# nghiapq77/face-recognition-cpp-tensorrt

Measured on AMD Instinct MI355X. Metric: faces/sec end-to-end (detect+embed+match), 640x640 batch=32, 1M gallery, higher is better.
Workload: dtype f16 MFMA recogniser convs (fp32 accumulate) + fp32-accurate detector (fp32 MFMA, fp16 hi/lo-split MFMA for the 64-channel 3x3 convs) + int8-screened coarse scan (fp16 MFMA on exactly widened int8 rows) + exact f32 re-rank match (bit-identical to the exact f32 scan)

## Files before the change

### face-recognition-cpp-tensorrt_amd/csrc/frt_kernels.h

```cpp
#pragma once
#include <hip/hip_runtime.h>
#include <stdint.h>

#include <vector>

#include "../../include/frt.h"
#include "frt_faces.hpp"

typedef _Float16 half_t;
typedef _Float16 half8 __attribute__((ext_vector_type(8)));
typedef _Float16 half4 __attribute__((ext_vector_type(4)));
typedef float floatx16 __attribute__((ext_vector_type(16)));
typedef float floatx4 __attribute__((ext_vector_type(4)));

constexpr int FRT_MAX_DEVICES = 32;
inline bool frt_first_use_on_device(bool (&done)[FRT_MAX_DEVICES]) {
    int d = 0;
    (void)hipGetDevice(&d);
    d &= FRT_MAX_DEVICES - 1;
    if (done[d]) return false;
    done[d] = true;
    return true;
}

// ... 230 lines not shown
    int linear;
    int nt;
    int R;
    int n_img;
    int nslot;
    int threads;
};
struct StripTables {
    int period = 0;
    int ppx = 0;
    int stride = 0;
    std::vector<int> data;
};
constexpr int strip_table_stride(const StripGeometry &g) { return g.nslot * g.threads + g.nt * 64 + (g.compact ? g.nt * 4 : g.nt * 32); }
StripTables strip_tables(const StripGeometry &g);
enum ConvFamily { CONV_SMALL, CONV_KS, CONV_C64, CONV_S2, CONV_STRIP };
struct ConvPlan {
    int family = CONV_STRIP;
    int row = 0;
    const char *label = "";
    int R = 0, n_img = 1;
    int M = 0;
    bool uses_scx = false;
    int se_row = -1;
    const char *se_label = nullptr;
    bool se_fused() const { return se_row >= 0; }
    void take_se_tail() { row = se_row; label = se_label; }
};
struct ConvRow {
    const char *label;
// ... 1 lines not shown
    int se_row;
};
inline void conv_plan_row(ConvPlan &p, int family, const ConvRow *table, int row) {
    p.family = family;
    p.row = row;
    p.label = table[row].label;
}
inline void conv_plan_se_twin(ConvPlan &p, const ConvRow *table, const ConvMfmaArgs &a) {
    if (table[p.row].se_row < 0 || a.mode != EPI_BN_ADD_BN || !a.se_pool || !a.sc || !a.out1) return;
    p.se_row = table[p.row].se_row;
    p.se_label = table[p.se_row].label;
}
ConvPlan conv_plan(const ConvMfmaArgs &a);
bool conv_strip_geometry(const ConvMfmaArgs &a, const ConvPlan &p, StripGeometry &g);
void conv_strip_tables_warm(const ConvMfmaArgs &a, const ConvPlan &p);
void launch_conv_mfma(const ConvMfmaArgs &a, const ConvPlan &p, hipStream_t s);
bool conv_se_fits_device();
bool plan_small(const ConvMfmaArgs &a, ConvPlan &p);
void launch_small(const ConvMfmaArgs &a, const ConvPlan &p, hipStream_t s);
bool plan_ks(const ConvMfmaArgs &a, ConvPlan &p);
void launch_ks(const ConvMfmaArgs &a, const ConvPlan &p, hipStream_t s);
bool plan_c64(const ConvMfmaArgs &a, ConvPlan &p);
void launch_c64(const ConvMfmaArgs &a, const ConvPlan &p, hipStream_t s);
bool plan_s2(const ConvMfmaArgs &a, ConvPlan &p);
void launch_s2(const ConvMfmaArgs &a, const ConvPlan &p, hipStream_t s);
struct ArcInputArgs {
    const float *x;
    const float *w;
    const float *s0, *b0;
    const float *slope;
// ... 37 lines not shown
```

### face-recognition-cpp-tensorrt_amd/csrc/kernels_arc.hip

```cpp
#include "frt_kernels.h"
#include "frt_se_device.h"

#include <array>
#include <map>
#include <mutex>
#include <stdexcept>
#include <string>
#include <type_traits>
#include <utility>
#include <vector>

namespace {

__device__ __forceinline__ int swz(int row, int chunk) { return chunk ^ ((row >> 1) & 7); }

template <int WCO, int WPX, int NSTAGE>
__global__ __launch_bounds__(256) void conv_glds_kernel(ConvMfmaArgs p) {
    constexpr int BCO = WCO * 64, BPX = WPX * 64;
    constexpr int CO_CH = BCO * 8 / 256, PX_CH = BPX * 8 / 256;
    constexpr int LPT = CO_CH + PX_CH;
    constexpr int STAGE_HALFS = (BCO + BPX) * 64;
    extern __shared__ __attribute__((aligned(16))) char smem[];
    half_t *ring = reinterpret_cast<half_t *>(smem);

// ... 878 lines not shown
    if (plan_c64(a, p)) return p;
    if (plan_s2(a, p)) return p;
    plan_strip(a, p);
    return p;
}

bool conv_strip_geometry(const ConvMfmaArgs &a, const ConvPlan &p, StripGeometry &g) {
    if (p.family != CONV_STRIP || !kStripGeometry[p.row]) return false;
    g = kStripGeometry[p.row](a, p);
    return true;
}

void conv_strip_tables_warm(const ConvMfmaArgs &a, const ConvPlan &p) {
    StripGeometry g;
    if (conv_strip_geometry(a, p, g)) (void)strip_tab_device(g);
}

StripTables strip_tables(const StripGeometry &g) {
    const int H = g.H, W = g.W, NT = g.nt, R = g.R, T = g.threads, P = H * W, S = NT * 32;
    auto bad = [](const char *what) { throw std::runtime_error(std::string("strip tables: ") + what); };
    if (H < 1 || W < 1 || NT < 1 || R < 1 || g.n_img < 1 || g.nslot < 1 || (T != 128 && T != 256)) bad("geometry");
    StripTables t;
    t.stride = strip_table_stride(g);
    const int o_pbase = g.nslot * T, o_tail = o_pbase + NT * 64;
    const int patch_bytes = g.nslot * T * 16, PROW = 144;
    const int Wp = g.compact ? W : W + 2;
    if (g.compact) {
        int a = P, b = S;
        while (b) { const int c = a % b; a = b; b = c; }
        t.period = P / a;
// ... 128 lines not shown
```

### face-recognition-cpp-tensorrt_amd/csrc/kernels_arc_s2.hip

```cpp
#include "frt_kernels.h"
#include "frt_se_device.h"

#include <type_traits>

namespace {

constexpr int PROW = 144;

__device__ constexpr int kSub[9] = {0, 0, 0, 0, 1, 2, 2, 3, 3};
__device__ constexpr int kDr[9] = {0, 0, 1, 1, 0, 0, 1, 0, 0};
__device__ constexpr int kDc[9] = {0, 1, 0, 1, 0, 0, 0, 0, 1};
__device__ constexpr int kLen[4] = {4, 1, 2, 2};
__device__ constexpr int kRowPar[4] = {1, 0, 1, 0};
__device__ constexpr int kColPar[4] = {1, 0, 0, 1};

template <int NT, int PP, bool SEP = false, bool SCF = false>
__global__ __launch_bounds__(256, 1) void conv_s2_kernel(ConvMfmaArgs p, int R, int n_img, int linear) {
    constexpr int PLANE_B = PP * 4096;
    constexpr int LA = 2, WR = 3, BFD = 2;
    extern __shared__ __attribute__((aligned(16))) char smem[];
    const int tid = threadIdx.x, lane = tid & 63, wave = tid >> 6;
    const int r = lane & 31, hi = lane >> 5;
    const int H = p.H, W = p.W, Ho = p.Ho, Wo = p.Wo, Wq = Wo + 1;
    const int NPp = n_img * (R + 1) * Wq;
    const int strips_per_img = Ho / R;
    const int n_valid = n_img * R * Wo;

    const int n_co_tiles = p.Cout >> 7;
    const int nblk = gridDim.x, bq = nblk >> 3, brem = nblk & 7;
    const int xcd = blockIdx.x & 7, slot = blockIdx.x >> 3;
    const int lid = (xcd < brem ? xcd * (bq + 1) : brem * (bq + 1) + (xcd - brem) * bq) + slot;
    const int co_tile = lid % n_co_tiles, strip = lid / n_co_tiles;
    const int co_base = co_tile * 128, cow = wave * 32;
    const int img0 = (strip / strips_per_img) * n_img;
    const int oy0 = (strip % strips_per_img) * R;
    const int n_chunks = p.Cin >> 6;

    int poff[4][PP];
    const int n_sc = SCF ? (p.Csc >> 6) : 0;
    int poff_sc[SCF ? PP : 1];
    {
        const int plane_px = (R + 1) * Wq;
        const float inv_plane = 1.0f / (float)plane_px, inv_row = 1.0f / (float)Wq;
#pragma unroll
        for (int q = 0; q < PP; ++q) {
            const int g = (q * 4 + wave) * 64 + lane;
            const int px = g / 9, pos = g - px * 9;
            int il = (int)(((float)px + 0.5f) * inv_plane);
            int rem = px - il * plane_px;
            if (rem < 0) { --il; rem += plane_px; } else if (rem >= plane_px) { ++il; rem -= plane_px; }
            int i = (int)(((float)rem + 0.5f) * inv_row);
            int j = rem - i * Wq;
            if (j < 0) { --i; j += Wq; } else if (j >= Wq) { ++i; j -= Wq; }
            const int b = img0 + il;
            const bool live = pos < 8 && px < NPp && b < p.B;
            const int ye = 2 * (oy0 + i), xe = 2 * j;
#pragma unroll
            for (int s = 0; s < 4; ++s) {
                const int y = ye - kRowPar[s], x = xe - kColPar[s];
                poff[s][q] = (live && y >= 0 && y < H && x >= 0 && x < W) ? ((b * H + y) * W + x) * p.Cin + pos * 8 : -1;
            }
            if constexpr (SCF) poff_sc[q] = (live && ye < H && xe < W) ? ((b * H + ye) * W + xe) * p.Csc + pos * 8 : -1;
        }
    }
    const half_t *wfrag = p.wf + ((long)((co_base + cow) >> 5) * n_chunks) * (9 * 4 * 512) + lane * 8;
    int pbase[NT];
#pragma unroll
    for (int j = 0; j < NT; ++j) {
        const int sl = j * 32 + r;
        int pidx = 0;
        if (linear) {
            pidx = sl < R * Wq ? sl : 0;
        } else if (sl < n_valid) {
            const int per = R * Wo;
            int il = (int)(((float)sl + 0.5f) * (1.0f / (float)per));
            int rem = sl - il * per;
            if (rem < 0) { --il; rem += per; } else if (rem >= per) { ++il; rem -= per; }
            int rr = (int)(((float)rem + 0.5f) * (1.0f / (float)Wo));
            int cc = rem - rr * Wo;
            if (cc < 0) { --rr; cc += Wo; } else if (cc >= Wo) { ++rr; cc -= Wo; }
            pidx = (il * (R + 1) + rr) * Wq + cc;
        }
        pbase[j] = pidx * PROW + hi * 16;
    }

    half8 areg[WR][4];
    auto load_w = [&](int c, int step, auto slot_c) {
        constexpr int S = decltype(slot_c)::value;
        const int woff = c < n_chunks ? (c * 9 + step) * (4 * 512) : 0;
#pragma unroll
        for (int kk = 0; kk < 4; ++kk) areg[S][kk] = *reinterpret_cast<const half8 *>(wfrag + woff + kk * 512);
    };
    auto issue_plane = [&](int c, auto sub_c) {
        constexpr int S = decltype(sub_c)::value;
        const bool real = c < n_chunks;
        char *pl = smem + S * PLANE_B + wave * 1024;
#pragma unroll
        for (int q = 0; q < PP; ++q) {
            const half_t *src = (real && poff[S][q] >= 0) ? p.x + (unsigned)(poff[S][q] + (c << 6)) : p.zeros;
            if constexpr (SCF) {
                if (!real && S < n_sc && poff_sc[q] >= 0) src = p.scx + (unsigned)(poff_sc[q] + (S << 6));
            }
            __builtin_amdgcn_global_load_lds((const __attribute__((address_space(1))) void *)src,
                                             (__attribute__((address_space(3))) void *)(pl + q * 4096), 16, 0, 0);
        }
    };

    floatx16 acc[NT];
#pragma unroll
    for (int j = 0; j < NT; ++j)
#pragma unroll
        for (int e = 0; e < 16; ++e) acc[j][e] = 0.f;

    issue_plane(0, std::integral_constant<int, 0>{});
    issue_plane(0, std::integral_constant<int, 1>{});
    issue_plane(0, std::integral_constant<int, 2>{});
    issue_plane(0, std::integral_constant<int, 3>{});
    load_w(0, 0, std::integral_constant<int, 0>{});
    load_w(0, 1, std::integral_constant<int, 1>{});
    half8 bf[BFD][NT];
    asm volatile("s_waitcnt vmcnt(%0)" ::"n"(4 * LA) : "memory");
    __builtin_amdgcn_s_barrier();
#pragma unroll
    for (int k2 = 0; k2 < BFD; ++k2)
#pragma unroll
        for (int j = 0; j < NT; ++j) bf[k2][j] = *reinterpret_cast<const half8 *>(smem + pbase[j] + k2 * 32);

    auto step = [&](int c, auto step_c) {
        constexpr int ST = decltype(step_c)::value;
        constexpr int NS = (ST + 1) % 9;
        constexpr int AS = ST % WR;
        constexpr bool LAST_OF_PLANE = kSub[NS] != kSub[ST];
        const int dp = kSub[ST] * PLANE_B + (kDr[ST] * Wq + kDc[ST]) * PROW;
        const int dpn = kSub[NS] * PLANE_B + (kDr[NS] * Wq + kDc[NS]) * PROW;
#pragma unroll
        for (int kk = 0; kk < 4; ++kk) {
            const int cur = kk & 1;
            if (kk == 4 - BFD && LAST_OF_PLANE) {
                constexpr int NEXT = kSub[NS];
                constexpr int YOUNGER = 4 * (9 - kLen[NEXT]) + 2 * PP;
                static_assert(YOUNGER <= 63, "vmcnt field");
                asm volatile("s_waitcnt vmcnt(%0)" ::"n"(YOUNGER) : "memory");
                asm volatile("s_waitcnt lgkmcnt(0)" ::: "memory");
                __builtin_amdgcn_s_barrier();
                __builtin_amdgcn_sched_barrier(0);
                issue_plane(c + 1, std::integral_constant<int, kSub[ST]>{});
                __builtin_amdgcn_sched_barrier(0);
            }
#pragma unroll
            for (int j = 0; j < NT; ++j) {
                acc[j] = __builtin_amdgcn_mfma_f32_32x32x16_f16(areg[AS][kk], bf[cur][j], acc[j], 0, 0, 0);
                if (kk + BFD < 4) bf[cur][j] = *reinterpret_cast<const half8 *>(smem + pbase[j] + dp + (kk + BFD) * 32);
                else bf[cur][j] = *reinterpret_cast<const half8 *>(smem + pbase[j] + dpn + (kk + BFD - 4) * 32);
                if (kk == 0 && j == (NT > 1 ? 1 : 0)) {
                    constexpr int T2 = ST + LA;
                    load_w(T2 < 9 ? c : c + 1, T2 % 9, std::integral_constant<int, (T2 % 9) % WR>{});
                }
                __builtin_amdgcn_sched_barrier(0);
            }
        }
    };
    for (int c = 0; c < n_chunks; ++c) {
        step(c, std::integral_constant<int, 0>{});
        step(c, std::integral_constant<int, 1>{});
        step(c, std::integral_constant<int, 2>{});
        step(c, std::integral_constant<int, 3>{});
        step(c, std::integral_constant<int, 4>{});
        step(c, std::integral_constant<int, 5>{});
        step(c, std::integral_constant<int, 6>{});
        step(c, std::integral_constant<int, 7>{});
        step(c, std::integral_constant<int, 8>{});
    }
    floatx16 acc_sc[SCF ? NT : 1];
    if constexpr (SCF) {
        half8 wsc[4][4];
        const half_t *wsf = p.wscf + ((long)((co_base + cow) >> 5) * n_sc) * (4 * 512) + lane * 8;
#pragma unroll
        for (int c = 0; c < 4; ++c)
#pragma unroll
            for (int kk = 0; kk < 4; ++kk) wsc[c][kk] = *reinterpret_cast<const half8 *>(wsf + ((c < n_sc ? c : 0) * 4 + kk) * 512);
#pragma unroll
        for (int j = 0; j < NT; ++j)
#pragma unroll
            for (int e = 0; e < 16; ++e) acc_sc[j][e] = 0.f;
        asm volatile("s_waitcnt vmcnt(0)" ::: "memory");
        __syncthreads();
#pragma unroll
        for (int c = 0; c < 4; ++c) {
            if (c < n_sc) {
#pragma unroll
                for (int kk = 0; kk < 4; ++kk)
#pragma unroll
                    for (int j = 0; j < NT; ++j) {
                        const half8 b = *reinterpret_cast<const half8 *>(smem + pbase[j] + c * PLANE_B + kk * 32);
                        acc_sc[j] = __builtin_amdgcn_mfma_f32_32x32x16_f16(wsc[c][kk], b, acc_sc[j], 0, 0, 0);
                    }
            }
        }
    } else {
        asm volatile("s_waitcnt vmcnt(0)" ::: "memory");
    }
    __syncthreads();

    constexpr int EROW = 36;
    float *ep = reinterpret_cast<float *>(smem) + wave * (32 * EROW);
    const int chunk = lane & 3;
    const int cch = co_base + cow + chunk * 8;
    floatx4 q0[2], q1[2], q2[2], q3[2];
    q0[0] = *reinterpret_cast<const floatx4 *>(p.p0 + cch);
    q0[1] = *reinterpret_cast<const floatx4 *>(p.p0 + cch + 4);
    q1[0] = *reinterpret_cast<const floatx4 *>(p.p1 + cch);
    q1[1] = *reinterpret_cast<const floatx4 *>(p.p1 + cch + 4);
    const bool two = p.mode == EPI_BN_ADD_BN && p.out1;
    if (two) {
        q2[0] = *reinterpret_cast<const floatx4 *>(p.p2 + cch);
        q2[1] = *reinterpret_cast<const floatx4 *>(p.p2 + cch + 4);
        q3[0] = *reinterpret_cast<const floatx4 *>(p.p3 + cch);
        q3[1] = *reinterpret_cast<const floatx4 *>(p.p3 + cch + 4);
    }
    const long Mtot = (long)p.B * Ho * Wo;
    const float inv_wq = 1.0f / (float)Wq;
    auto slot_pixel = [&](int sl, long &m) -> bool {
        if (linear) {
            const int rr = (int)(((float)sl + 0.5f) * inv_wq);
            const int cc = sl - rr * Wq;
            m = ((long)img0 * Ho + oy0 + rr) * Wo + cc;
            return rr < R && cc < Wo && m < Mtot;
        }
        m = ((long)img0 * Ho + oy0) * Wo + sl;
        return sl < n_valid && m < Mtot;
    };
    if constexpr (SEP) {
        const int per_img = R * Wo;
        se_tail_epilogue<NT, (NT == 4 ? 2 : 1)>(p, acc, ep, reinterpret_cast<float *>(smem + 4 * 32 * EROW * 4), strip % strips_per_img, strips_per_img,
                                               n_co_tiles, img0, n_img, Ho * Wo, co_base, cow, [&](int sl, long &m, int &il) -> bool {
                                                   il = (NT == 4 && !linear && sl >= per_img) ? 1 : 0;
                                                   return slot_pixel(sl, m);
                                               });
        return;
    }
    half8 sc8[SCF ? 1 : NT][2];
    floatx4 qs0[2], qs1[2];
    if constexpr (SCF) {
        qs0[0] = *reinterpret_cast<const floatx4 *>(p.psc0 + cch);
        qs0[1] = *reinterpret_cast<const floatx4 *>(p.psc0 + cch + 4);
        qs1[0] = *reinterpret_cast<const floatx4 *>(p.psc1 + cch);
        qs1[1] = *reinterpret_cast<const floatx4 *>(p.psc1 + cch + 4);
    } else if (p.mode == EPI_BN_ADD_BN) {
#pragma unroll
        for (int j = 0; j < NT; ++j)
#pragma unroll
            for (int it = 0; it < 2; ++it) {
                const int sl = j * 32 + (lane >> 2) + 16 * it;
                long m;
                const bool ok = slot_pixel(sl, m);
                sc8[j][it] = *reinterpret_cast<const half8 *>(p.sc + (ok ? m : 0) * p.Cout + cch);
            }
    }
#pragma unroll
    for (int j = 0; j < NT; ++j) {
        float v[2][8];
#pragma unroll
        for (int g = 0; g < 4; ++g) {
            const floatx4 t = {acc[j][4 * g], acc[j][4 * g + 1], acc[j][4 * g + 2], acc[j][4 * g + 3]};
            *reinterpret_cast<floatx4 *>(ep + r * EROW + 8 * g + 4 * hi) = t;
        }
#pragma unroll
        for (int it = 0; it < 2; ++it) {
            const int px = (lane >> 2) + 16 * it;
            const floatx4 v0 = *reinterpret_cast<const floatx4 *>(ep + px * EROW + chunk * 8);
            const floatx4 v1 = *reinterpret_cast<const floatx4 *>(ep + px * EROW + chunk * 8 + 4);
            const float t[8] = {v0[0], v0[1], v0[2], v0[3], v1[0], v1[1], v1[2], v1[3]};
#pragma unroll
            for (int e = 0; e < 8; ++e) v[it][e] = t[e] * q0[e >> 2][e & 3] + q1[e >> 2][e & 3];
        }
        if constexpr (SCF) {
#pragma unroll
            for (int g = 0; g < 4; ++g) {
                const floatx4 t = {acc_sc[j][4 * g], acc_sc[j][4 * g + 1], acc_sc[j][4 * g + 2], acc_sc[j][4 * g + 3]};
                *reinterpret_cast<floatx4 *>(ep + r * EROW + 8 * g + 4 * hi) = t;
            }
#pragma unroll
            for (int it = 0; it < 2; ++it) {
                const int px = (lane >> 2) + 16 * it;
                const floatx4 v0 = *reinterpret_cast<const floatx4 *>(ep + px * EROW + chunk * 8);
                const floatx4 v1 = *reinterpret_cast<const floatx4 *>(ep + px * EROW + chunk * 8 + 4);
                const float t[8] = {v0[0], v0[1], v0[2], v0[3], v1[0], v1[1], v1[2], v1[3]};
#pragma unroll
                for (int e = 0; e < 8; ++e) v[it][e] += t[e] * qs0[e >> 2][e & 3] + qs1[e >> 2][e & 3];
            }
        } else if (p.mode == EPI_BN_ADD_BN) {
#pragma unroll
            for (int it = 0; it < 2; ++it)
#pragma unroll
                for (int e = 0; e < 8; ++e) v[it][e] += (float)sc8[j][it][e];
        }
#pragma unroll
        for (int it = 0; it < 2; ++it) {
            const int sl = j * 32 + (lane >> 2) + 16 * it;
            long m;
            if (!slot_pixel(sl, m)) continue;
            half8 o;
#pragma unroll
            for (int e = 0; e < 8; ++e) o[e] = (half_t)v[it][e];
            *reinterpret_cast<half8 *>(p.out0 + m * p.Cout + cch) = o;
            if (two) {
                half8 z;
#pragma unroll
                for (int e = 0; e < 8; ++e) z[e] = (half_t)(v[it][e] * q2[e >> 2][e & 3] + q3[e >> 2][e & 3]);
                *reinterpret_cast<half8 *>(p.out1 + m * p.Cout + cch) = z;
            }
        }
    }
}
// ... 145 lines not shown
                }
            }
        }
        if (two) asm volatile("s_waitcnt vmcnt(8)" ::: "memory");
        else asm volatile("s_waitcnt vmcnt(4)" ::: "memory");
    }
}

bool s2c64_applies(const ConvMfmaArgs &a) {
    if (!a.wf2 || a.ks != 3 || a.stride != 2 || a.pad != 1 || a.Cout != 64 || a.Cin != 64 || a.splits != 1 || (a.H & 1) || (a.W & 1)) return false;
    if (a.Ho * 2 != a.H || a.Wo * 2 != a.W || a.Wo != 56 || a.Ho != 56) return false;
    if (a.mode != EPI_BN && a.mode != EPI_BN_ADD_BN) return false;
    return a.mode != EPI_BN_ADD_BN || a.sc;
}

template <int NT, int PP, bool SEP = false, bool SCF = false>
void launch_s2_t(const ConvMfmaArgs &a0, const ConvPlan &p, hipStream_t s) {
    constexpr size_t lds = (size_t)4 * PP * 4096;
    static_assert(lds <= 160 * 1024 && lds >= 4 * 32 * 36 * 4, "LDS budget / epilogue scratch");
    static bool attr_done[FRT_MAX_DEVICES] = {};
    if (frt_first_use_on_device(attr_done))
        (void)hipFuncSetAttribute(reinterpret_cast<const void *>(&conv_s2_kernel<NT, PP, SEP, SCF>), hipFuncAttributeMaxDynamicSharedMemorySize, (int)lds);
    ConvMfmaArgs a = a0;
    a.wf = a0.wf2;
    const int strips = ((a.B + p.n_img - 1) / p.n_img) * (a.Ho / p.R);
    const int linear = (p.n_img == 1 && p.R * (a.Wo + 1) <= NT * 32) ? 1 : 0;
    hipLaunchKernelGGL((conv_s2_kernel<NT, PP, SEP, SCF>), dim3(strips * (a.Cout / 128)), dim3(256), lds, s, a, p.R, p.n_img, linear);
}

void launch_s2c64(const ConvMfmaArgs &a0, const ConvPlan &, hipStream_t s) {
    ConvMfmaArgs a = a0;
    a.wf = a0.wf2;
    static bool attr_done[FRT_MAX_DEVICES] = {};
    if (frt_first_use_on_device(attr_done))
        (void)hipFuncSetAttribute(reinterpret_cast<const void *>(&conv_s2c64_kernel), hipFuncAttributeMaxDynamicSharedMemorySize, C64_LDS);
    const int n_rows = a.B * a.Ho;
    hipLaunchKernelGGL(conv_s2c64_kernel, dim3(n_rows < 768 ? n_rows : 768), dim3(128), C64_LDS, s, a, n_rows);
}

bool s2_geometry(const ConvMfmaArgs &a, int &R, int &n_img, int &nt, int &pp) {
    if (!a.wf2 || a.ks != 3 || a.stride != 2 || a.pad != 1 || a.Cout % 128 || a.Cin % 64 || a.splits != 1 || a.H != a.W || (a.H & 1)) return false;
    if (a.Ho * 2 != a.H || a.Wo * 2 != a.W) return false;
// ... 7 lines not shown
        n_img = (a.B >= 96 && 2 * a.Ho * a.Wo <= 128) ? 2 : 1;
        nt = n_img * a.Ho * a.Wo <= 64 ? 2 : 4;
    } else {
        n_img = 1;
        R = 0;
        for (int d = a.Ho; d >= 1; --d) {
            if (a.Ho % d || d * Wq > 224) continue;
            R = d;
            break;
        }
        if (!R) return false;
        nt = R * Wq <= 128 ? 4 : 7;
        if (R * a.Wo * 10 < nt * 32 * 7) return false;
    }
    pp = (n_img * (R + 1) * Wq * 9 + 255) / 256;
    return pp <= 9;
}

enum { S2_C64, S2_7, S2_7_SCF, S2_7_SE, S2_4, S2_4_SCF, S2_4_SE, S2_4W, S2_4W_SCF, S2_2, S2_2_SCF };
const ConvRow kS2[] = {
     {"conv_s2c64_kernel", launch_s2c64, -1},
     {"conv_s2_kernel<7, 9, false, false>", launch_s2_t<7, 9>, S2_7_SE},
     {"conv_s2_kernel<7, 9, false, true>", launch_s2_t<7, 9, false, true>, -1},
     {"conv_s2_kernel<7, 9, true, false>", launch_s2_t<7, 9, true>, -1},
     {"conv_s2_kernel<4, 5, false, false>", launch_s2_t<4, 5>, S2_4_SE},
     {"conv_s2_kernel<4, 5, false, true>", launch_s2_t<4, 5, false, true>, -1},
     {"conv_s2_kernel<4, 5, true, false>", launch_s2_t<4, 5, true>, -1},
     {"conv_s2_kernel<4, 9, false, false>", launch_s2_t<4, 9>, -1},
     {"conv_s2_kernel<4, 9, false, true>", launch_s2_t<4, 9, false, true>, -1},
     {"conv_s2_kernel<2, 5, false, false>", launch_s2_t<2, 5>, -1},
     {"conv_s2_kernel<2, 5, false, true>", launch_s2_t<2, 5, false, true>, -1},
};

}

bool plan_s2(const ConvMfmaArgs &a, ConvPlan &p) {
    if (s2c64_applies(a)) {
        conv_plan_row(p, CONV_S2, kS2, S2_C64);
        return true;
    }
    int R, n_img, nt, pp;
    if (!s2_geometry(a, R, n_img, nt, pp)) return false;
    const bool scf = a.mode == EPI_BN_ADD_BN && a.scx;
    const int base = nt == 7 ? S2_7 : (nt == 4 ? (pp <= 5 ? S2_4 : S2_4W) : S2_2);
    conv_plan_row(p, CONV_S2, kS2, base + (scf ? 1 : 0));
    p.R = R;
    p.n_img = n_img;
    p.uses_scx = scf;
    const bool se_geom = nt == 7 ? (n_img == 1 && a.Ho / R <= SE_SPLIT) : (n_img == 2 ? R == a.Ho : (n_img == 1 && a.Ho / R <= SE_SPLIT));
    if (se_geom) conv_plan_se_twin(p, kS2, a);
    return true;
}

void launch_s2(const ConvMfmaArgs &a, const ConvPlan &p, hipStream_t s) { kS2[p.row].launch(a, p, s); }
```

Before: 43990.

## Use precomputed offset tables and a two-plane LDS ring in stride-2 conv

The stride-2 strip conv kernel now reads per-strip gather offsets, B-fragment bases and epilogue pixel offsets from host-built device tables, replacing the in-kernel float-division index math and the 4xPP offset registers with one packed offset plus a live-bit mask. For large-plane instantiations (PP>5, non-SE) the four sub-plane LDS buffers become a two-plane ring, and BN parameters are staged in LDS. This roughly halves LDS use so two workgroups fit per CU (launch bounds raised to 2). The shortcut GEMM is moved after the main loop for ring variants. Costs are extra table loads, a narrower prefetch window, tighter vmcnt scheduling, and new limits (Csc<=128, 32-bit offsets).

```diff
diff --git a/face-recognition-cpp-tensorrt_amd/csrc/frt_kernels.h b/face-recognition-cpp-tensorrt_amd/csrc/frt_kernels.h
--- a/face-recognition-cpp-tensorrt_amd/csrc/frt_kernels.h
+++ b/face-recognition-cpp-tensorrt_amd/csrc/frt_kernels.h
@@ -268,6 +268,21 @@
 };
 constexpr int strip_table_stride(const StripGeometry &g) { return g.nslot * g.threads + g.nt * 64 + (g.compact ? g.nt * 4 : g.nt * 32); }
 StripTables strip_tables(const StripGeometry &g);
+struct S2Geometry {
+    int H;
+    int R;
+    int n_img;
+    int nt;
+    int pp;
+    int linear;
+};
+struct S2Tables {
+    int period = 0;
+    int stride = 0;
+    std::vector<int> data;
+};
+constexpr int s2_table_stride(const S2Geometry &g) { return g.pp * 256 + g.nt * 96; }
+S2Tables s2_tables(const S2Geometry &g);
 enum ConvFamily { CONV_SMALL, CONV_KS, CONV_C64, CONV_S2, CONV_STRIP };
 struct ConvPlan {
     int family = CONV_STRIP;
@@ -299,6 +314,8 @@
 ConvPlan conv_plan(const ConvMfmaArgs &a);
 bool conv_strip_geometry(const ConvMfmaArgs &a, const ConvPlan &p, StripGeometry &g);
 void conv_strip_tables_warm(const ConvMfmaArgs &a, const ConvPlan &p);
+bool conv_s2_geometry(const ConvMfmaArgs &a, const ConvPlan &p, S2Geometry &g);
+void conv_s2_tables_warm(const ConvMfmaArgs &a, const ConvPlan &p);
 void launch_conv_mfma(const ConvMfmaArgs &a, const ConvPlan &p, hipStream_t s);
 bool conv_se_fits_device();
 bool plan_small(const ConvMfmaArgs &a, ConvPlan &p);
diff --git a/face-recognition-cpp-tensorrt_amd/csrc/kernels_arc.hip b/face-recognition-cpp-tensorrt_amd/csrc/kernels_arc.hip
--- a/face-recognition-cpp-tensorrt_amd/csrc/kernels_arc.hip
+++ b/face-recognition-cpp-tensorrt_amd/csrc/kernels_arc.hip
@@ -916,6 +916,7 @@
 void conv_strip_tables_warm(const ConvMfmaArgs &a, const ConvPlan &p) {
     StripGeometry g;
     if (conv_strip_geometry(a, p, g)) (void)strip_tab_device(g);
+    conv_s2_tables_warm(a, p);
 }
 
 StripTables strip_tables(const StripGeometry &g) {
diff --git a/face-recognition-cpp-tensorrt_amd/csrc/kernels_arc_s2.hip b/face-recognition-cpp-tensorrt_amd/csrc/kernels_arc_s2.hip
--- a/face-recognition-cpp-tensorrt_amd/csrc/kernels_arc_s2.hip
+++ b/face-recognition-cpp-tensorrt_amd/csrc/kernels_arc_s2.hip
@@ -1,11 +1,23 @@
 #include "frt_kernels.h"
 #include "frt_se_device.h"
 
+#include <array>
+#include <map>
+#include <mutex>
+#include <stdexcept>
+#include <string>
 #include <type_traits>
+#include <utility>
+#include <vector>
 
 namespace {
 
 constexpr int PROW = 144;
+
+constexpr bool s2_ring(int pp, bool sep) { return !sep && pp > 5; }
+constexpr bool s2_two_per_cu(int pp, bool sep) { return !sep; }
+constexpr int S2_PRM_BYTES = 6 * 128 * 4;
+constexpr size_t s2_lds_bytes(int pp, bool sep) { return s2_ring(pp, sep) ? (size_t)2 * pp * 4096 + S2_PRM_BYTES : (size_t)4 * pp * 4096; }
 
 __device__ constexpr int kSub[9] = {0, 0, 0, 0, 1, 2, 2, 3, 3};
 __device__ constexpr int kDr[9] = {0, 0, 1, 1, 0, 0, 1, 0, 0};
@@ -15,16 +27,15 @@
 __device__ constexpr int kColPar[4] = {1, 0, 0, 1};
 
 template <int NT, int PP, bool SEP = false, bool SCF = false>
-__global__ __launch_bounds__(256, 1) void conv_s2_kernel(ConvMfmaArgs p, int R, int n_img, int linear) {
+__global__ __launch_bounds__(256, s2_two_per_cu(PP, SEP) ? 2 : 1) void conv_s2_kernel(ConvMfmaArgs p, int R, int n_img, int linear) {
     constexpr int PLANE_B = PP * 4096;
-    constexpr int LA = 2, WR = 3, BFD = 2;
+    constexpr bool RING = s2_ring(PP, SEP);
+    constexpr int LA = (RING && SCF && NT == 7) ? 1 : 2, WR = 3, BFD = RING ? 1 : 2;
+    auto buf_of = [](int plane) constexpr { return RING ? (plane & 1) : plane; };
     extern __shared__ __attribute__((aligned(16))) char smem[];
     const int tid = threadIdx.x, lane = tid & 63, wave = tid >> 6;
-    const int r = lane & 31, hi = lane >> 5;
     const int H = p.H, W = p.W, Ho = p.Ho, Wo = p.Wo, Wq = Wo + 1;
-    const int NPp = n_img * (R + 1) * Wq;
     const int strips_per_img = Ho / R;
-    const int n_valid = n_img * R * Wo;
 
     const int n_co_tiles = p.Cout >> 7;
     const int nblk = gridDim.x, bq = nblk >> 3, brem = nblk & 7;
@@ -33,56 +44,34 @@
     const int co_tile = lid % n_co_tiles, strip = lid / n_co_tiles;
     const int co_base = co_tile * 128, cow = wave * 32;
     const int img0 = (strip / strips_per_img) * n_img;
-    const int oy0 = (strip % strips_per_img) * R;
     const int n_chunks = p.Cin >> 6;
 
-    int poff[4][PP];
+    constexpr int T_STRIDE = PP * 256 + NT * 96;
+    const int *__restrict__ tab = p.strip_tab + (strip % strips_per_img) * T_STRIDE;
+    unsigned poff[PP];
+    unsigned pmask[(PP + 5) / 6];
+#pragma unroll
+    for (int i = 0; i < (PP + 5) / 6; ++i) pmask[i] = 0;
+    auto plive = [&](int q, int bit) -> bool { return (pmask[q / 6] >> ((q % 6) * 5 + bit)) & 1; };
     const int n_sc = SCF ? (p.Csc >> 6) : 0;
-    int poff_sc[SCF ? PP : 1];
+    int poff_sc[(SCF && !RING) ? PP : 1];
     {
-        const int plane_px = (R + 1) * Wq;
-        const float inv_plane = 1.0f / (float)plane_px, inv_row = 1.0f / (float)Wq;
+        const int px0 = img0 * (H * W);
 #pragma unroll
         for (int q = 0; q < PP; ++q) {
-            const int g = (q * 4 + wave) * 64 + lane;
-            const int px = g / 9, pos = g - px * 9;
-            int il = (int)(((float)px + 0.5f) * inv_plane);
-            int rem = px - il * plane_px;
-            if (rem < 0) { --il; rem += plane_px; } else if (rem >= plane_px) { ++il; rem -= plane_px; }
-            int i = (int)(((float)rem + 0.5f) * inv_row);
-            int j = rem - i * Wq;
-            if (j < 0) { --i; j += Wq; } else if (j >= Wq) { ++i; j -= Wq; }
-            const int b = img0 + il;
-            const bool live = pos < 8 && px < NPp && b < p.B;
-            const int ye = 2 * (oy0 + i), xe = 2 * j;
-#pragma unroll
-            for (int s = 0; s < 4; ++s) {
-                const int y = ye - kRowPar[s], x = xe - kColPar[s];
-                poff[s][q] = (live && y >= 0 && y < H && x >= 0 && x < W) ? ((b * H + y) * W + x) * p.Cin + pos * 8 : -1;
-            }
-            if constexpr (SCF) poff_sc[q] = (live && ye < H && xe < W) ? ((b * H + ye) * W + xe) * p.Csc + pos * 8 : -1;
+            const int t = tab[q * 256 + tid];
+            const bool live = t >= 0 && img0 + ((t >> 8) & 15) < p.B;
+            const int px = px0 + (t >> 12), pos8 = ((t >> 5) & 7) * 8;
+            pmask[q / 6] |= live ? (unsigned)(t & 31) << ((q % 6) * 5) : 0u;
+            poff[q] = (unsigned)(px * p.Cin + pos8);
+            if constexpr (SCF && !RING) poff_sc[q] = px * p.Csc + pos8;
         }
     }
     const half_t *wfrag = p.wf + ((long)((co_base + cow) >> 5) * n_chunks) * (9 * 4 * 512) + lane * 8;
     int pbase[NT];
 #pragma unroll
-    for (int j = 0; j < NT; ++j) {
-        const int sl = j * 32 + r;
-        int pidx = 0;
-        if (linear) {
-            pidx = sl < R * Wq ? sl : 0;
-        } else if (sl < n_valid) {
-            const int per = R * Wo;
-            int il = (int)(((float)sl + 0.5f) * (1.0f / (float)per));
-            int rem = sl - il * per;
-            if (rem < 0) { --il; rem += per; } else if (rem >= per) { ++il; rem -= per; }
-            int rr = (int)(((float)rem + 0.5f) * (1.0f / (float)Wo));
-            int cc = rem - rr * Wo;
-            if (cc < 0) { --rr; cc += Wo; } else if (cc >= Wo) { ++rr; cc -= Wo; }
-            pidx = (il * (R + 1) + rr) * Wq + cc;
-        }
-        pbase[j] = pidx * PROW + hi * 16;
-    }
+    for (int j = 0; j < NT; ++j) pbase[j] = tab[PP * 256 + j * 64 + lane];
+    const int *__restrict__ eoff = tab + PP * 256 + NT * 64;
 
     half8 areg[WR][4];
     auto load_w = [&](int c, int step, auto slot_c) {
@@ -91,18 +80,21 @@
 #pragma unroll
         for (int kk = 0; kk < 4; ++kk) areg[S][kk] = *reinterpret_cast<const half8 *>(wfrag + woff + kk * 512);
     };
+    int cin = p.Cin;
     auto issue_plane = [&](int c, auto sub_c) {
         constexpr int S = decltype(sub_c)::value;
         const bool real = c < n_chunks;
-        char *pl = smem + S * PLANE_B + wave * 1024;
+        char *pl = smem + buf_of(S) * PLANE_B + wave * 1024;
+        const unsigned d = (unsigned)((c << 6) - (kRowPar[S] * W + kColPar[S]) * cin);
 #pragma unroll
         for (int q = 0; q < PP; ++q) {
-            const half_t *src = (real && poff[S][q] >= 0) ? p.x + (unsigned)(poff[S][q] + (c << 6)) : p.zeros;
-            if constexpr (SCF) {
-                if (!real && S < n_sc && poff_sc[q] >= 0) src = p.scx + (unsigned)(poff_sc[q] + (S << 6));
+            const half_t *src = (real && plive(q, S)) ? p.x + (poff[q] + d) : p.zeros;
+            if constexpr (SCF && !RING) {
+                if (!real && S < n_sc && plive(q, 4)) src = p.scx + (unsigned)(poff_sc[q] + (S << 6));
             }
             __builtin_amdgcn_global_load_lds((const __attribute__((address_space(1))) void *)src,
                                              (__attribute__((address_space(3))) void *)(pl + q * 4096), 16, 0, 0);
+            if constexpr (RING) __builtin_amdgcn_sched_barrier(0);
         }
     };
 
@@ -112,39 +104,55 @@
 #pragma unroll
         for (int e = 0; e < 16; ++e) acc[j][e] = 0.f;
 
-    issue_plane(0, std::integral_constant<int, 0>{});
-    issue_plane(0, std::integral_constant<int, 1>{});
-    issue_plane(0, std::integral_constant<int, 2>{});
-    issue_plane(0, std::integral_constant<int, 3>{});
-    load_w(0, 0, std::integral_constant<int, 0>{});
-    load_w(0, 1, std::integral_constant<int, 1>{});
     half8 bf[BFD][NT];
-    asm volatile("s_waitcnt vmcnt(%0)" ::"n"(4 * LA) : "memory");
+    if constexpr (RING) {
+        issue_plane(0, std::integral_constant<int, 0>{});
+        load_w(0, 0, std::integral_constant<int, 0>{});
+        if constexpr (LA == 2) load_w(0, 1, std::integral_constant<int, 1>{});
+        issue_plane(0, std::integral_constant<int, 1>{});
+        static_assert(4 * LA + PP <= 63, "vmcnt field");
+        asm volatile("s_waitcnt vmcnt(%0)" ::"n"(4 * LA + PP) : "memory");
+    } else {
+        issue_plane(0, std::integral_constant<int, 0>{});
+        issue_plane(0, std::integral_constant<int, 1>{});
+        issue_plane(0, std::integral_constant<int, 2>{});
+        issue_plane(0, std::integral_constant<int, 3>{});
+        load_w(0, 0, std::integral_constant<int, 0>{});
+        load_w(0, 1, std::integral_constant<int, 1>{});
+        asm volatile("s_waitcnt vmcnt(%0)" ::"n"(4 * LA) : "memory");
+    }
     __builtin_amdgcn_s_barrier();
 #pragma unroll
     for (int k2 = 0; k2 < BFD; ++k2)
 #pragma unroll
         for (int j = 0; j < NT; ++j) bf[k2][j] = *reinterpret_cast<const half8 *>(smem + pbase[j] + k2 * 32);
 
+    int wq = Wq;
     auto step = [&](int c, auto step_c) {
         constexpr int ST = decltype(step_c)::value;
         constexpr int NS = (ST + 1) % 9;
         constexpr int AS = ST % WR;
         constexpr bool LAST_OF_PLANE = kSub[NS] != kSub[ST];
-        const int dp = kSub[ST] * PLANE_B + (kDr[ST] * Wq + kDc[ST]) * PROW;
-        const int dpn = kSub[NS] * PLANE_B + (kDr[NS] * Wq + kDc[NS]) * PROW;
+        const int dp = buf_of(kSub[ST]) * PLANE_B + (kDr[ST] * wq + kDc[ST]) * PROW;
+        const int dpn = buf_of(kSub[NS]) * PLANE_B + (kDr[NS] * wq + kDc[NS]) * PROW;
 #pragma unroll
         for (int kk = 0; kk < 4; ++kk) {
-            const int cur = kk & 1;
+            const int cur = kk % BFD;
             if (kk == 4 - BFD && LAST_OF_PLANE) {
-                constexpr int NEXT = kSub[NS];
-                constexpr int YOUNGER = 4 * (9 - kLen[NEXT]) + 2 * PP;
+                constexpr int CUR = kSub[ST], NEXT = kSub[NS];
+                constexpr int YOUNGER = RING ? 4 * kLen[CUR] : 4 * (9 - kLen[NEXT]) + 2 * PP;
                 static_assert(YOUNGER <= 63, "vmcnt field");
                 asm volatile("s_waitcnt vmcnt(%0)" ::"n"(YOUNGER) : "memory");
                 asm volatile("s_waitcnt lgkmcnt(0)" ::: "memory");
                 __builtin_amdgcn_s_barrier();
                 __builtin_amdgcn_sched_barrier(0);
-                issue_plane(c + 1, std::integral_constant<int, kSub[ST]>{});
+                if constexpr (RING) {
+                    const int rc = c + (CUR >= 2 ? 1 : 0);
+                    if (rc < n_chunks) issue_plane(rc, std::integral_constant<int, (CUR + 2) % 4>{});
+
+                } else {
+                    issue_plane(c + 1, std::integral_constant<int, CUR>{});
+                }
                 __builtin_amdgcn_sched_barrier(0);
             }
 #pragma unroll
@@ -161,6 +169,10 @@
         }
     };
     for (int c = 0; c < n_chunks; ++c) {
+        wq = Wq;
+        cin = p.Cin;
+        if constexpr (RING) asm volatile("" : "+s"(wq), "+s"(cin));
+
         step(c, std::integral_constant<int, 0>{});
         step(c, std::integral_constant<int, 1>{});
         step(c, std::integral_constant<int, 2>{});
@@ -171,10 +183,71 @@
         step(c, std::integral_constant<int, 7>{});
         step(c, std::integral_constant<int, 8>{});
     }
-    floatx16 acc_sc[SCF ? NT : 1];
-    if constexpr (SCF) {
+    int tid_e = tid;
+    if constexpr (RING) asm volatile("" : "+v"(tid_e));
+    if constexpr (RING && SCF) {
+#pragma unroll
+        for (int i = 0; i < (PP + 5) / 6; ++i) asm volatile("" : "+v"(pmask[i]));
+    }
+    const int lane_e = tid_e & 63, wave_e = tid_e >> 6, r_e = lane_e & 31, hi_e = lane_e >> 5, cow_e = wave_e * 32;
+    auto issue_sc_plane = [&](int sc) {
+        char *pl = smem + sc * PLANE_B + wave_e * 1024;
+#pragma unroll
+        for (int q = 0; q < PP; ++q) {
+            const int t = tab[q * 256 + tid_e];
+            const half_t *src = plive(q, 4) ? p.scx + (unsigned)((img0 * (H * W) + (t >> 12)) * p.Csc + ((t >> 5) & 7) * 8 + (sc << 6)) : p.zeros;
+            __builtin_amdgcn_global_load_lds((const __attribute__((address_space(1))) void *)src,
+                                             (__attribute__((address_space(3))) void *)(pl + q * 4096), 16, 0, 0);
+        }
+    };
+
+    float *prm = reinterpret_cast<float *>(smem + 2 * PLANE_B);
+    const bool two = p.mode == EPI_BN_ADD_BN && p.out1;
+    if constexpr (RING) {
+        if (tid_e < 128) {
+            const int co = co_base + tid_e;
+            prm[tid_e] = p.p0[co];
+            prm[128 + tid_e] = p.p1[co];
+            if (two) prm[256 + tid_e] = p.p2[co], prm[384 + tid_e] = p.p3[co];
+            if constexpr (SCF) prm[512 + tid_e] = p.psc0[co], prm[640 + tid_e] = p.psc1[co];
+        }
+    }
+    constexpr bool SC_TILE = SCF && RING;
+    floatx16 acc_sc[(SCF && !RING) ? NT : 1];
+    half8 wsc2[SC_TILE ? 2 : 1][4];
+    auto sc_tile = [&](int j) -> floatx16 {
+        floatx16 a;
+#pragma unroll
+        for (int e = 0; e < 16; ++e) a[e] = 0.f;
+#pragma unroll
+        for (int c = 0; c < 2; ++c) {
+            if (c < n_sc) {
+#pragma unroll
+                for (int kk = 0; kk < 4; ++kk) {
+                    const half8 b = *reinterpret_cast<const half8 *>(smem + pbase[j] + c * PLANE_B + kk * 32);
+                    a = __builtin_amdgcn_mfma_f32_32x32x16_f16(wsc2[SC_TILE ? c : 0][kk], b, a, 0, 0, 0);
+                }
+            }
+        }
+        return a;
+    };
+    floatx16 acc_s0;
+    if constexpr (SC_TILE) {
+        const half_t *wsf = p.wscf + ((long)((co_base + cow_e) >> 5) * n_sc) * (4 * 512) + lane_e * 8;
+#pragma unroll
+        for (int c = 0; c < 2; ++c)
+#pragma unroll
+            for (int kk = 0; kk < 4; ++kk) wsc2[c][kk] = *reinterpret_cast<const half8 *>(wsf + ((c < n_sc ? c : 0) * 4 + kk) * 512);
+        __syncthreads();
+#pragma unroll
+        for (int c = 0; c < 2; ++c)
+            if (c < n_sc) issue_sc_plane(c);
+        asm volatile("s_waitcnt vmcnt(0)" ::: "memory");
+        __syncthreads();
+        acc_s0 = sc_tile(0);
+    } else if constexpr (SCF) {
         half8 wsc[4][4];
-        const half_t *wsf = p.wscf + ((long)((co_base + cow) >> 5) * n_sc) * (4 * 512) + lane * 8;
+        const half_t *wsf = p.wscf + ((long)((co_base + cow_e) >> 5) * n_sc) * (4 * 512) + lane_e * 8;
 #pragma unroll
         for (int c = 0; c < 4; ++c)
 #pragma unroll
@@ -203,101 +276,168 @@
     __syncthreads();
 
     constexpr int EROW = 36;
-    float *ep = reinterpret_cast<float *>(smem) + wave * (32 * EROW);
-    const int chunk = lane & 3;
-    const int cch = co_base + cow + chunk * 8;
-    floatx4 q0[2], q1[2], q2[2], q3[2];
-    q0[0] = *reinterpret_cast<const floatx4 *>(p.p0 + cch);
-    q0[1] = *reinterpret_cast<const floatx4 *>(p.p0 + cch + 4);
-    q1[0] = *reinterpret_cast<const floatx4 *>(p.p1 + cch);
-    q1[1] = *reinterpret_cast<const floatx4 *>(p.p1 + cch + 4);
-    const bool two = p.mode == EPI_BN_ADD_BN && p.out1;
-    if (two) {
-        q2[0] = *reinterpret_cast<const floatx4 *>(p.p2 + cch);
-        q2[1] = *reinterpret_cast<const floatx4 *>(p.p2 + cch + 4);
-        q3[0] = *reinterpret_cast<const floatx4 *>(p.p3 + cch);
-        q3[1] = *reinterpret_cast<const floatx4 *>(p.p3 + cch + 4);
-    }
+    const int chunk = lane_e & 3;
+    const int cch = co_base + cow_e + chunk * 8;
     const long Mtot = (long)p.B * Ho * Wo;
-    const float inv_wq = 1.0f / (float)Wq;
+    const long m_base = (long)img0 * Ho * Wo;
     auto slot_pixel = [&](int sl, long &m) -> bool {
-        if (linear) {
-            const int rr = (int)(((float)sl + 0.5f) * inv_wq);
-            const int cc = sl - rr * Wq;
-            m = ((long)img0 * Ho + oy0 + rr) * Wo + cc;
-            return rr < R && cc < Wo && m < Mtot;
-        }
-        m = ((long)img0 * Ho + oy0) * Wo + sl;
-        return sl < n_valid && m < Mtot;
-    };
+        const int e = eoff[sl];
+        m = m_base + e;
+        return e >= 0 && m < Mtot;
+    };
+    if constexpr (RING) {
+        float *ep = reinterpret_cast<float *>(smem + (wave_e & 1) * PLANE_B + (wave_e >> 1) * (16 * EROW * 4));
+        const float *prl = prm + cow_e + chunk * 8;
+        auto half_through = [&](const floatx16 &a, int it, float (&t)[8]) {
+            if ((r_e >> 4) == it) {
+#pragma unroll
+                for (int g = 0; g < 4; ++g) {
+                    const floatx4 w4 = {a[4 * g], a[4 * g + 1], a[4 * g + 2], a[4 * g + 3]};
+                    *reinterpret_cast<floatx4 *>(ep + (r_e & 15) * EROW + 8 * g + 4 * hi_e) = w4;
+                }
+            }
+            asm volatile("" ::: "memory");
+            const floatx4 v0 = *reinterpret_cast<const floatx4 *>(ep + (lane_e >> 2) * EROW + chunk * 8);
+            const floatx4 v1 = *reinterpret_cast<const floatx4 *>(ep + (lane_e >> 2) * EROW + chunk * 8 + 4);
+#pragma unroll
+            for (int e = 0; e < 4; ++e) t[e] = v0[e], t[4 + e] = v1[e];
+        };
+        auto param8 = [&](int which, float (&q)[8]) {
+            const floatx4 a = *reinterpret_cast<const floatx4 *>(prl + which * 128), b = *reinterpret_cast<const floatx4 *>(prl + which * 128 + 4);
+#pragma unroll
+            for (int e = 0; e < 4; ++e) q[e] = a[e], q[4 + e] = b[e];
+        };
+        const bool add_sc = !SCF && p.mode == EPI_BN_ADD_BN;
+        half8 sc8[2][2];
+        auto load_sc = [&](int j) {
+#pragma unroll
+            for (int it = 0; it < 2; ++it) {
+                const int sl = j * 32 + (lane_e >> 2) + 16 * it;
+                long m;
+                const bool ok = slot_pixel(sl, m);
+                sc8[j & 1][it] = *reinterpret_cast<const half8 *>(p.sc + (ok ? m : 0) * p.Cout + cch);
+            }
+        };
+        if (add_sc) load_sc(0);
+#pragma unroll
+        for (int j = 0; j < NT; ++j) {
+            floatx16 a_sc;
+            if constexpr (SCF) a_sc = j == 0 ? acc_s0 : sc_tile(j);
+            if (add_sc && j + 1 < NT) load_sc(j + 1);
+#pragma unroll
+            for (int it = 0; it < 2; ++it) {
+                asm volatile("" ::: "memory");
+                float t[8], v[8], qa[8], qb[8];
+                half_through(acc[j], it, t);
+                param8(0, qa);
+                param8(1, qb);
+#pragma unroll
+                for (int e = 0; e < 8; ++e) v[e] = t[e] * qa[e] + qb[e];
+                if constexpr (SCF) {
+                    half_through(a_sc, it, t);
+                    param8(4, qa);
+                    param8(5, qb);
+#pragma unroll
+                    for (int e = 0; e < 8; ++e) v[e] += t[e] * qa[e] + qb[e];
+                } else if (add_sc) {
+#pragma unroll
+                    for (int e = 0; e < 8; ++e) v[e] += (float)sc8[j & 1][it][e];
+                }
+                const int sl = j * 32 + (lane_e >> 2) + 16 * it;
+                long m;
+                if (!slot_pixel(sl, m)) continue;
+                half8 o;
+#pragma unroll
+                for (int e = 0; e < 8; ++e) o[e] = (half_t)v[e];
+                *reinterpret_cast<half8 *>(p.out0 + m * p.Cout + cch) = o;
+                if (two) {
+                    param8(2, qa);
+                    param8(3, qb);
+                    half8 z;
+#pragma unroll
+                    for (int e = 0; e < 8; ++e) z[e] = (half_t)(v[e] * qa[e] + qb[e]);
+                    *reinterpret_cast<half8 *>(p.out1 + m * p.Cout + cch) = z;
+                }
+            }
+        }
+        return;
+    }
+    float *ep = reinterpret_cast<float *>(smem) + wave_e * (32 * EROW);
+    auto through_lds = [&](const floatx16 &a, float (&t)[2][8]) {
+#pragma unroll
+        for (int g = 0; g < 4; ++g) {
+            const floatx4 w4 = {a[4 * g], a[4 * g + 1], a[4 * g + 2], a[4 * g + 3]};
+            *reinterpret_cast<floatx4 *>(ep + r_e * EROW + 8 * g + 4 * hi_e) = w4;
+        }
+#pragma unroll
+        for (int it = 0; it < 2; ++it) {
+            const int px = (lane_e >> 2) + 16 * it;
+            const floatx4 v0 = *reinterpret_cast<const floatx4 *>(ep + px * EROW + chunk * 8);
+            const floatx4 v1 = *reinterpret_cast<const floatx4 *>(ep + px * EROW + chunk * 8 + 4);
+#pragma unroll
+            for (int e = 0; e < 4; ++e) t[it][e] = v0[e], t[it][4 + e] = v1[e];
+        }
+    };
+    floatx4 q0[2], q1[2], q2[2], q3[2], qs0[2], qs1[2];
+#pragma unroll
+    for (int h = 0; h < 2; ++h) {
+        q0[h] = *reinterpret_cast<const floatx4 *>(p.p0 + cch + 4 * h);
+        q1[h] = *reinterpret_cast<const floatx4 *>(p.p1 + cch + 4 * h);
+        if (two) {
+            q2[h] = *reinterpret_cast<const floatx4 *>(p.p2 + cch + 4 * h);
+            q3[h] = *reinterpret_cast<const floatx4 *>(p.p3 + cch + 4 * h);
+        }
+        if constexpr (SCF) {
+            qs0[h] = *reinterpret_cast<const floatx4 *>(p.psc0 + cch + 4 * h);
+            qs1[h] = *reinterpret_cast<const floatx4 *>(p.psc1 + cch + 4 * h);
+        }
+    }
     if constexpr (SEP) {
         const int per_img = R * Wo;
         se_tail_epilogue<NT, (NT == 4 ? 2 : 1)>(p, acc, ep, reinterpret_cast<float *>(smem + 4 * 32 * EROW * 4), strip % strips_per_img, strips_per_img,
-                                               n_co_tiles, img0, n_img, Ho * Wo, co_base, cow, [&](int sl, long &m, int &il) -> bool {
+                                               n_co_tiles, img0, n_img, Ho * Wo, co_base, cow_e, [&](int sl, long &m, int &il) -> bool {
                                                    il = (NT == 4 && !linear && sl >= per_img) ? 1 : 0;
                                                    return slot_pixel(sl, m);
                                                });
         return;
     }
     half8 sc8[SCF ? 1 : NT][2];
-    floatx4 qs0[2], qs1[2];
-    if constexpr (SCF) {
-        qs0[0] = *reinterpret_cast<const floatx4 *>(p.psc0 + cch);
-        qs0[1] = *reinterpret_cast<const floatx4 *>(p.psc0 + cch + 4);
-        qs1[0] = *reinterpret_cast<const floatx4 *>(p.psc1 + cch);
-        qs1[1] = *reinterpret_cast<const floatx4 *>(p.psc1 + cch + 4);
-    } else if (p.mode == EPI_BN_ADD_BN) {
-#pragma unroll
-        for (int j = 0; j < NT; ++j)
-#pragma unroll
-            for (int it = 0; it < 2; ++it) {
-                const int sl = j * 32 + (lane >> 2) + 16 * it;
-                long m;
-                const bool ok = slot_pixel(sl, m);
-                sc8[j][it] = *reinterpret_cast<const half8 *>(p.sc + (ok ? m : 0) * p.Cout + cch);
-            }
+    if constexpr (!SCF) {
+        if (p.mode == EPI_BN_ADD_BN) {
+#pragma unroll
+            for (int j = 0; j < NT; ++j)
+#pragma unroll
+                for (int it = 0; it < 2; ++it) {
+                    const int sl = j * 32 + (lane_e >> 2) + 16 * it;
+                    long m;
+                    const bool ok = slot_pixel(sl, m);
+                    sc8[j][it] = *reinterpret_cast<const half8 *>(p.sc + (ok ? m : 0) * p.Cout + cch);
+                }
+        }
     }
 #pragma unroll
     for (int j = 0; j < NT; ++j) {
-        float v[2][8];
-#pragma unroll
-        for (int g = 0; g < 4; ++g) {
-            const floatx4 t = {acc[j][4 * g], acc[j][4 * g + 1], acc[j][4 * g + 2], acc[j][4 * g + 3]};
-            *reinterpret_cast<floatx4 *>(ep + r * EROW + 8 * g + 4 * hi) = t;
+        float v[2][8], t[2][8];
+        through_lds(acc[j], t);
+#pragma unroll
+        for (int it = 0; it < 2; ++it)
+#pragma unroll
+            for (int e = 0; e < 8; ++e) v[it][e] = t[it][e] * q0[e >> 2][e & 3] + q1[e >> 2][e & 3];
+        if constexpr (SCF) {
+            through_lds(acc_sc[j], t);
+#pragma unroll
+            for (int it = 0; it < 2; ++it)
+#pragma unroll
+                for (int e = 0; e < 8; ++e) v[it][e] += t[it][e] * qs0[e >> 2][e & 3] + qs1[e >> 2][e & 3];
+        } else if (p.mode == EPI_BN_ADD_BN) {
+#pragma unroll
+            for (int it = 0; it < 2; ++it)
+#pragma unroll
+                for (int e = 0; e < 8; ++e) v[it][e] += (float)sc8[j][it][e];
         }
 #pragma unroll
         for (int it = 0; it < 2; ++it) {
-            const int px = (lane >> 2) + 16 * it;
-            const floatx4 v0 = *reinterpret_cast<const floatx4 *>(ep + px * EROW + chunk * 8);
-            const floatx4 v1 = *reinterpret_cast<const floatx4 *>(ep + px * EROW + chunk * 8 + 4);
-            const float t[8] = {v0[0], v0[1], v0[2], v0[3], v1[0], v1[1], v1[2], v1[3]};
-#pragma unroll
-            for (int e = 0; e < 8; ++e) v[it][e] = t[e] * q0[e >> 2][e & 3] + q1[e >> 2][e & 3];
-        }
-        if constexpr (SCF) {
-#pragma unroll
-            for (int g = 0; g < 4; ++g) {
-                const floatx4 t = {acc_sc[j][4 * g], acc_sc[j][4 * g + 1], acc_sc[j][4 * g + 2], acc_sc[j][4 * g + 3]};
-                *reinterpret_cast<floatx4 *>(ep + r * EROW + 8 * g + 4 * hi) = t;
-            }
-#pragma unroll
-            for (int it = 0; it < 2; ++it) {
-                const int px = (lane >> 2) + 16 * it;
-                const floatx4 v0 = *reinterpret_cast<const floatx4 *>(ep + px * EROW + chunk * 8);
-                const floatx4 v1 = *reinterpret_cast<const floatx4 *>(ep + px * EROW + chunk * 8 + 4);
-                const float t[8] = {v0[0], v0[1], v0[2], v0[3], v1[0], v1[1], v1[2], v1[3]};
-#pragma unroll
-                for (int e = 0; e < 8; ++e) v[it][e] += t[e] * qs0[e >> 2][e & 3] + qs1[e >> 2][e & 3];
-            }
-        } else if (p.mode == EPI_BN_ADD_BN) {
-#pragma unroll
-            for (int it = 0; it < 2; ++it)
-#pragma unroll
-                for (int e = 0; e < 8; ++e) v[it][e] += (float)sc8[j][it][e];
-        }
-#pragma unroll
-        for (int it = 0; it < 2; ++it) {
-            const int sl = j * 32 + (lane >> 2) + 16 * it;
+            const int sl = j * 32 + (lane_e >> 2) + 16 * it;
             long m;
             if (!slot_pixel(sl, m)) continue;
             half8 o;
@@ -473,18 +613,54 @@
     return a.mode != EPI_BN_ADD_BN || a.sc;
 }
 
+const int *s2_tab_device(const S2Geometry &g, hipStream_t s = nullptr) {
+    static std::mutex mu;
+    static std::map<std::array<int, 7>, const int *> cache;
+    thread_local std::vector<std::pair<std::array<int, 7>, const int *>> mine;
+    int d = 0;
+    (void)hipGetDevice(&d);
+    const std::array<int, 7> key = {d, g.H, g.R, g.n_img, g.nt, g.pp, g.linear};
+    for (const auto &e : mine)
+        if (e.first == key) return e.second;
+    std::lock_guard<std::mutex> lock(mu);
+    auto it = cache.find(key);
+    if (it == cache.end()) {
+        hipStreamCaptureStatus cap = hipStreamCaptureStatusNone;
+        if (s && hipStreamIsCapturing(s, &cap) == hipSuccess && cap != hipStreamCaptureStatusNone)
+            throw std::runtime_error("stride-2 strip tables: first use of a strip geometry inside a stream capture (frt_embedder::build() warms every geometry it plans)");
+        const S2Tables t = s2_tables(g);
+        int *dev = nullptr;
+        if (hipMalloc(reinterpret_cast<void **>(&dev), t.data.size() * sizeof(int)) != hipSuccess ||
+            hipMemcpy(dev, t.data.data(), t.data.size() * sizeof(int), hipMemcpyHostToDevice) != hipSuccess)
+            throw std::runtime_error("stride-2 strip tables: device allocation or copy failed");
+        it = cache.emplace(key, dev).first;
+    }
+    mine.emplace_back(key, it->second);
+    return it->second;
+}
+template <int NT, int PP>
+S2Geometry s2_strip_geometry(const ConvMfmaArgs &a, const ConvPlan &p) {
+    const int linear = (p.n_img == 1 && p.R * (a.Wo + 1) <= NT * 32) ? 1 : 0;
+    return S2Geometry{a.H, p.R, p.n_img, NT, PP, linear};
+}
+
 template <int NT, int PP, bool SEP = false, bool SCF = false>
 void launch_s2_t(const ConvMfmaArgs &a0, const ConvPlan &p, hipStream_t s) {
-    constexpr size_t lds = (size_t)4 * PP * 4096;
+    constexpr size_t lds = s2_lds_bytes(PP, SEP);
     static_assert(lds <= 160 * 1024 && lds >= 4 * 32 * 36 * 4, "LDS budget / epilogue scratch");
+    static_assert(!s2_two_per_cu(PP, SEP) || 2 * lds <= 160 * 1024, "two workgroups per CU");
     static bool attr_done[FRT_MAX_DEVICES] = {};
     if (frt_first_use_on_device(attr_done))
         (void)hipFuncSetAttribute(reinterpret_cast<const void *>(&conv_s2_kernel<NT, PP, SEP, SCF>), hipFuncAttributeMaxDynamicSharedMemorySize, (int)lds);
+    if ((long)a0.B * a0.H * a0.W * a0.Cin >= (1L << 31) || (SCF && (long)a0.B * a0.H * a0.W * a0.Csc >= (1L << 31)))
+        throw std::runtime_error("stride-2 strip kernel: an input tensor exceeds 32-bit element offsets");
+    if (SCF && s2_ring(PP, SEP) && a0.Csc > 128) throw std::runtime_error("stride-2 strip kernel: the ring instantiations park at most two shortcut chunks");
+    const S2Geometry g = s2_strip_geometry<NT, PP>(a0, p);
     ConvMfmaArgs a = a0;
     a.wf = a0.wf2;
+    a.strip_tab = s2_tab_device(g, s);
     const int strips = ((a.B + p.n_img - 1) / p.n_img) * (a.Ho / p.R);
-    const int linear = (p.n_img == 1 && p.R * (a.Wo + 1) <= NT * 32) ? 1 : 0;
-    hipLaunchKernelGGL((conv_s2_kernel<NT, PP, SEP, SCF>), dim3(strips * (a.Cout / 128)), dim3(256), lds, s, a, p.R, p.n_img, linear);
+    hipLaunchKernelGGL((conv_s2_kernel<NT, PP, SEP, SCF>), dim3(strips * (a.Cout / 128)), dim3(256), lds, s, a, p.R, p.n_img, g.linear);
 }
 
 void launch_s2c64(const ConvMfmaArgs &a0, const ConvPlan &, hipStream_t s) {
@@ -522,6 +698,7 @@
         if (R * a.Wo * 10 < nt * 32 * 7) return false;
     }
     pp = (n_img * (R + 1) * Wq * 9 + 255) / 256;
+    if (scf && (nt == 7 || pp > 5) && a.Csc > 128) return false;
     return pp <= 9;
 }
 
@@ -540,6 +717,22 @@
      {"conv_s2_kernel<2, 5, false, true>", launch_s2_t<2, 5, false, true>, -1},
 };
 
+typedef S2Geometry (*S2GeometryFn)(const ConvMfmaArgs &, const ConvPlan &);
+const S2GeometryFn kS2Geometry[] = {
+     nullptr,
+     s2_strip_geometry<7, 9>,
+     s2_strip_geometry<7, 9>,
+     s2_strip_geometry<7, 9>,
+     s2_strip_geometry<4, 5>,
+     s2_strip_geometry<4, 5>,
+     s2_strip_geometry<4, 5>,
+     s2_strip_geometry<4, 9>,
+     s2_strip_geometry<4, 9>,
+     s2_strip_geometry<2, 5>,
+     s2_strip_geometry<2, 5>,
+};
+static_assert(sizeof(kS2Geometry) / sizeof(kS2Geometry[0]) == sizeof(kS2) / sizeof(kS2[0]), "one geometry per row");
+
 }
 
 bool plan_s2(const ConvMfmaArgs &a, ConvPlan &p) {
@@ -561,3 +754,81 @@
 }
 
 void launch_s2(const ConvMfmaArgs &a, const ConvPlan &p, hipStream_t s) { kS2[p.row].launch(a, p, s); }
+
+bool conv_s2_geometry(const ConvMfmaArgs &a, const ConvPlan &p, S2Geometry &g) {
+    if (p.family != CONV_S2 || !kS2Geometry[p.row]) return false;
+    g = kS2Geometry[p.row](a, p);
+    return true;
+}
+
+void conv_s2_tables_warm(const ConvMfmaArgs &a, const ConvPlan &p) {
+    S2Geometry g;
+    if (conv_s2_geometry(a, p, g)) (void)s2_tab_device(g);
+}
+
+S2Tables s2_tables(const S2Geometry &g) {
+    const int H = g.H, W = g.H, Ho = H / 2, Wo = W / 2, Wq = Wo + 1, NT = g.nt, R = g.R, PP = g.pp;
+    auto bad = [](const char *what) { throw std::runtime_error(std::string("stride-2 strip tables: ") + what); };
+    if (H < 2 || (H & 1) || NT < 1 || R < 1 || Ho % R || g.n_img < 1 || g.n_img > 16 || PP < 1 || (g.n_img > 1 && R != Ho) || (g.linear && g.n_img != 1)) bad("geometry");
+    const int plane_px = (R + 1) * Wq, NPp = g.n_img * plane_px, plane_bytes = PP * 4096, PROW = 144;
+    if (NPp * 9 > PP * 256) bad("the plane does not fit its buffer");
+    if (g.linear ? R * Wq > NT * 32 : g.n_img * R * Wo > NT * 32) bad("the strip's pixels do not fit its tiles");
+    static const int row_par[4] = {1, 0, 1, 0}, col_par[4] = {1, 0, 0, 1};
+    static const int dr[9] = {0, 0, 1, 1, 0, 0, 1, 0, 0}, dc[9] = {0, 1, 0, 1, 0, 0, 0, 0, 1};
+    S2Tables t;
+    t.period = Ho / R;
+    t.stride = s2_table_stride(g);
+    t.data.assign((size_t)t.period * t.stride, -1);
+    const int o_pbase = PP * 256, o_eoff = o_pbase + NT * 64;
+    for (int sp = 0; sp < t.period; ++sp) {
+        int *blk = t.data.data() + (size_t)sp * t.stride;
+        const int oy0 = sp * R;
+        for (int piece = 0; piece < PP * 256; ++piece) {
+            const int px = piece / 9, pos = piece % 9;
+            if (pos == 8 || px >= NPp) continue;
+            const int il = px / plane_px, rem = px % plane_px, ye = 2 * (oy0 + rem / Wq), xe = 2 * (rem % Wq);
+            const int e = (il * H + ye) * W + xe;
+            int mask = 0;
+            for (int s = 0; s < 4; ++s) {
+                const int y = ye - row_par[s], x = xe - col_par[s];
+                if (y < 0 || y >= H || x < 0 || x >= W) continue;
+                const int at = e - row_par[s] * W - col_par[s];
+                if (at != (il * H + y) * W + x || at < il * H * W || at >= (il + 1) * H * W) bad("input pixel outside its image");
+                mask |= 1 << s;
+            }
+            if (ye < H && xe < W) mask |= 16;
+            if (!mask) continue;
+            if (e < 0 || e >= (1 << 19)) bad("input pixel outside the entry's field");
+            blk[piece] = (e << 12) | (il << 8) | (pos << 5) | mask;
+        }
+        for (int j = 0; j < NT; ++j)
+            for (int lane = 0; lane < 64; ++lane) {
+                const int sl = j * 32 + (lane & 31), hi = lane >> 5;
+                int pidx = 0;
+                if (g.linear) {
+                    pidx = sl < R * Wq ? sl : 0;
+                } else if (sl < g.n_img * R * Wo) {
+                    const int per = R * Wo, il = sl / per, r2 = sl % per;
+                    pidx = (il * (R + 1) + r2 / Wo) * Wq + r2 % Wo;
+                }
+                const int pb = pidx * PROW + hi * 16;
+                for (int st = 0; st < 9; ++st) {
+                    const int at = pb + (dr[st] * Wq + dc[st]) * PROW;
+                    if (at < 0 || at + 3 * 32 + 16 > plane_bytes) bad("B fragment outside the plane buffer");
+                }
+                blk[o_pbase + j * 64 + lane] = pb;
+            }
+        for (int sl = 0; sl < NT * 32; ++sl) {
+            int e = -1;
+            if (g.linear) {
+                const int rr = sl / Wq, cc = sl % Wq;
+                if (rr < R && cc < Wo) e = (oy0 + rr) * Wo + cc;
+            } else if (sl < g.n_img * R * Wo) {
+                e = oy0 * Wo + sl;
+            }
+            if (e < -1 || e >= g.n_img * Ho * Wo) bad("output pixel outside the image group");
+            blk[o_eoff + sl] = e;
+        }
+    }
+    return t;
+}
```

Result: no change. 44420 (median of 6 runs) (+1.0%).
